# lucagem29/mcmc_clv_model

Hardware: AMD Instinct MI355X
Metric: MCMC sweeps/sec x N_customers (customer-sweeps/s) (higher is better)
Workload: dtype f64

## Files before the change

include/clvmcmc.h:

```cpp
#ifndef CLVMCMC_H
#define CLVMCMC_H

#include <stdint.h>

#ifdef __cplusplus
extern "C" {
#endif

#define CLV_ABI_VERSION 2

#define CLV_BLOCK 256
#define CLV_MAX_K 9
#define CLV_MAX_D 3

enum { CLV_OK = 0, CLV_EINVAL = -1, CLV_EHIP = -2, CLV_ESTATE = -3, CLV_ENOMEM = -4 };
enum { CLV_RNG_PHILOX = 0, CLV_RNG_REPLAY = 1 };
enum { CLV_SINK_FULL = 0, CLV_SINK_SUMMARY = 1, CLV_SINK_NONE = 2, CLV_SINK_SUMMARY_PCT = 3 };

#define CLV_SUMMARY_MU_CAP 0.05
enum {
  CLV_SUM_LAMBDA = 0, CLV_SUM_MU, CLV_SUM_Z, CLV_SUM_LOG_LAMBDA, CLV_SUM_LOG_MU,
  CLV_SUM_LAMBDA2, CLV_SUM_MU2, CLV_SUM_ETA, CLV_SUM_LOG_ETA, CLV_SUM_MU_CAPPED, CLV_SUM_TAU,
  CLV_N_SUM_STATS
};
// ... 69 lines not shown
int clv_clock_probe(clv_sampler* s, double us, double* ghz);
int clv_launch_info(const clv_sampler* s, int64_t* out);
int clv_split_relay_steps(const clv_sampler* s, int32_t* out);
#define CLV_IPC_HANDLE_BYTES 64
int clv_p2p_info(const clv_sampler* s, int64_t* out);
int clv_p2p_export(clv_sampler* s, void* handle);
int clv_p2p_connect(clv_sampler* s, const void* handles, const uint64_t* ptrs);
int clv_p2p_disconnect(clv_sampler* s);
int clv_p2p_set_persistent(clv_sampler* s, int32_t on);
int clv_set_wait_timeout(clv_sampler* s, double ms);
int clv_set_stream(clv_sampler* s, uint64_t stream);
int clv_note_sweeps(clv_sampler* s, int64_t n);

int clv_read_draws(clv_sampler* s, double* level1, double* level2, double* loglik);
int clv_stream_draws(clv_sampler* s, double* level1);
int clv_read_summary(clv_sampler* s, double* sums, int64_t* n_stored);

int clv_get_state(clv_sampler* s, double* lambdas, double* mus, double* hyper);
int clv_set_state(clv_sampler* s, const double* lambdas, const double* mus, const double* hyper,
                  int64_t sweeps_done);

int clv_set_timing(clv_sampler* s, int32_t enable);
int clv_kernel_time(clv_sampler* s, double* sweep_kernel_ms_total, int64_t* sweep_launches,
                    double* hyper_kernel_ms_total, int64_t* hyper_launches);

int clv_debug_host_times(const clv_sampler* s, int64_t* out);
int clv_debug_philox(uint32_t k0, uint32_t k1, const uint32_t* ctr, int64_t n, uint32_t* out);
int clv_debug_variates(uint64_t seed, int32_t chain, uint32_t sweep, int64_t n, int32_t n_steps,
                       float* t_l, float* t_m, float* u_acc, double* u_z, double* u_tau,
                       double* e_alive, double* eta_z, float* log2_u_acc);
int clv_debug_log2u_scan(uint64_t w_begin, uint64_t w_end, double* out);
int clv_debug_t3(const uint32_t* words, int64_t n, int32_t packed, float* t_l, float* t_m);
int clv_debug_level2(int32_t D, int32_t K, const clv_prior* prior, const double* xty,
                     const double* yty, const double* iw_normal, const double* iw_chi2,
                     const double* z, double* beta, double* sigma);
int clv_debug_stamps(clv_sampler* s, uint64_t* out);
int clv_debug_wg_stamps(clv_sampler* s, uint64_t* out);
int clv_debug_hyper_variates(uint64_t seed, int32_t chain, uint32_t sweep, double df, int64_t n,
                             double* chi2, double* normals);
int clv_debug_exp(const double* x, int64_t n, double* out);
int clv_debug_log(const double* x, int64_t n, double* out);
int clv_debug_mh_step(int64_t n, const int32_t* x, const uint8_t* z, const double* T_cal, const double* tau,
                      const double* mean, const double* prec3, const double* cur_pt, const float* t3,
                      const double* scale2, const float* log_u, double* out);
int clv_debug_wg_map(int32_t n_chains, int32_t nb, int32_t n_cu, int32_t* out);
int clv_debug_persist_fits(int64_t grid_wgs, int32_t blocks_per_cu, int32_t n_cu);
int clv_debug_persist_choice(int32_t D, int32_t K, int32_t n_chains, int64_t grid_wgs, int32_t blocks_per_cu,
                             int32_t n_cu);
int clv_debug_split_fits(int32_t n_chains, int32_t nb, int32_t blocks_per_cu, int32_t n_cu);
int clv_debug_split_choice(int32_t n_chains, int32_t nb, int32_t blocks_per_cu, int32_t n_cu);
int clv_debug_split_layout(int32_t n_chains, int32_t nb, int32_t* out);
int clv_debug_split_relay_plan(int32_t S, int32_t R, int32_t* out);
int clv_debug_split_draw_plan(int32_t R, int32_t share, int32_t* out);
int clv_debug_split_stamps(clv_sampler* s, uint64_t* out);

enum { CLV_EXCHANGE_AUTO = 0, CLV_EXCHANGE_P2P = 1, CLV_EXCHANGE_COPY = 2 };
typedef struct clv_group clv_group;
int clv_group_create(clv_sampler* const* shards, int32_t n, int32_t exchange, clv_group** out);
int clv_group_run(clv_group* g, int64_t n_sweeps);
int32_t clv_group_exchange(const clv_group* g);
void clv_group_destroy(clv_group* g);

enum {
  CLV_L1_MEAN_LAMBDA = 0, CLV_L1_LAMBDA_P025, CLV_L1_LAMBDA_P975, CLV_L1_MEAN_MU, CLV_L1_MEAN_MU_CAPPED,
  CLV_L1_MU_P025, CLV_L1_MU_P975, CLV_L1_MEAN_Z, CLV_L1_MEAN_TAU, CLV_L1_MEAN_ETA, CLV_N_L1_STATS
};
int clv_predict(int32_t device, const double* level1, int64_t n_draws, int64_t n, int32_t width,
                const double* T_cal, double T_star, uint64_t seed, int32_t simulate_spend, double sigma_s,
                int64_t* x_future, double* spend_future);
int clv_predict_sampler(clv_sampler* s, double T_star, uint64_t seed, int32_t simulate_spend,
                        double sigma_s, int64_t* x_future, double* spend_future);
int clv_track(int32_t device, const double* level1, int64_t n_draws, int64_t n, int32_t width,
              const double* birth_week, const double* times, int32_t n_times, uint64_t seed,
              double* inc_weekly);
int clv_track_sampler(clv_sampler* s, const double* birth_week, const double* times, int32_t n_times,
                      uint64_t seed, double* inc_weekly);
int clv_level1_summary(int32_t device, const double* level1, int64_t n_draws, int64_t n, int32_t width,
                       double mu_cap, double* out);
int clv_level1_summary_sampler(clv_sampler* s, double mu_cap, double* out);
int clv_chain_total_loglik(int32_t device, const double* level1, int64_t n_draws, int64_t n, int32_t width,
                           const int32_t* x, const double* T_cal, double* mean_total);
int clv_chain_total_loglik_sampler(clv_sampler* s, double* mean_total);

enum {
  CLV_LTV_VALUE_MEAN = 0, CLV_LTV_VALUE_SD, CLV_LTV_VALUE_P025, CLV_LTV_VALUE_P50, CLV_LTV_VALUE_P975,
  CLV_LTV_RESIDUAL_MEAN, CLV_LTV_RESIDUAL_SD, CLV_LTV_RESIDUAL_P025, CLV_LTV_RESIDUAL_P50, CLV_LTV_RESIDUAL_P975,
  CLV_LTV_P_ALIVE, CLV_LTV_LIFETIME_YRS, CLV_LTV_SURVIVAL_1YR, CLV_N_LTV_STATS
};
enum {
  CLV_LTV_DRAW_EQUITY = 0, CLV_LTV_DRAW_VALUE_TOTAL, CLV_LTV_DRAW_N_ALIVE, CLV_LTV_DRAW_MU_SHARE,
  CLV_N_LTV_DRAW_STATS
};
int clv_lifetime_value(int32_t device, const double* level1, int64_t n_draws, int64_t n, int32_t width,
                       const double* monetary , double delta, double horizon ,
                       double value_scale, double periods_per_year, double* out_customers, double* out_draws);
int clv_lifetime_value_sampler(clv_sampler* s, const double* monetary, double delta, double horizon,
                               double value_scale, double periods_per_year, double* out_customers,
                               double* out_draws);
int clv_ltv_info(int64_t* out);

enum {
  CLV_IC_LPPD = 0, CLV_IC_P_WAIC, CLV_IC_ELPD_WAIC, CLV_IC_ELPD_LOO, CLV_IC_P_LOO, CLV_IC_PARETO_K,
  CLV_IC_TAIL_LEN, CLV_N_IC_STATS
};
int clv_pointwise_loglik(int32_t device, const double* level1, int64_t n_draws, int64_t n, int32_t width,
                         const int32_t* x, const double* t_x, const double* T_cal,
// ... 130 lines not shown
```

mcmc_clv_model_amd/_lib.py:

```python
from __future__ import annotations

import ctypes
import os
from ctypes import c_uint8, POINTER, c_char_p, c_double, c_float, c_int32, c_int64, c_uint32, c_uint64, c_void_p

try:
    import torch
except Exception:
    torch = None

LIB_NAME = "libclvmcmc.so"
LIB_PATH = os.environ.get("CLV_LIB_PATH") or os.path.join(os.path.dirname(os.path.abspath(__file__)), LIB_NAME)

ABI_VERSION = 2
BLOCK = 256
MAX_K = 9
MAX_D = 3
RNG_PHILOX, RNG_REPLAY = 0, 1
SINK_FULL, SINK_SUMMARY, SINK_NONE, SINK_SUMMARY_PCT = 0, 1, 2, 3
EXCHANGE_AUTO, EXCHANGE_P2P, EXCHANGE_COPY = 0, 1, 2
SUM_STATS = ("lambda", "mu", "z", "log_lambda", "log_mu", "lambda2", "mu2", "eta", "log_eta", "mu_capped", "tau")
SUMMARY_MU_CAP = 0.05
N_SUM_STATS = len(SUM_STATS)
TAPE_HYPER = 40
# ... 43 lines not shown
    L = ctypes.CDLL(LIB_PATH, mode=ctypes.RTLD_GLOBAL)
    sp = c_void_p
    dp = POINTER(c_double)
    sigs = {
        "clv_abi_version": (c_int32, []),
        "clv_default_blocks_per_unit": (c_int32, [c_int64]),
        "clv_sizeof": (c_int64, [c_int32]),
        "clv_last_error": (c_char_p, []),
        "clv_device_count": (c_int32, [POINTER(c_int32)]),
        "clv_create": (c_int32, [POINTER(ClvConfig), POINTER(ClvData), POINTER(ClvPrior), POINTER(sp)]),
        "clv_destroy": (None, [sp]),
        "clv_set_replay_tape": (c_int32, [sp, dp, c_int64]),
        "clv_replay_sweep_stride": (c_int64, [sp]),
        "clv_run": (c_int32, [sp, c_int64]),
        "clv_rollback": (c_int32, [sp]),
        "clv_sweep": (c_int32, [sp]),
        "clv_hyper": (c_int32, [sp, c_void_p]),
        "clv_partials": (c_int32, [sp, POINTER(c_void_p), POINTER(c_int64), POINTER(c_int32)]),
        "clv_copy_partials": (c_int32, [sp, c_void_p]),
        "clv_synchronize": (c_int32, [sp]),
        "clv_sweeps_done": (c_int64, [sp]),
        "clv_clock_ghz": (c_int32, [sp, POINTER(c_double)]),
        "clv_clock_probe": (c_int32, [sp, c_double, POINTER(c_double)]),
        "clv_launch_info": (c_int32, [sp, POINTER(c_int64)]),
        "clv_split_relay_steps": (c_int32, [sp, POINTER(c_int32)]),
        "clv_p2p_info": (c_int32, [sp, POINTER(c_int64)]),
        "clv_p2p_export": (c_int32, [sp, c_void_p]),
        "clv_p2p_connect": (c_int32, [sp, c_void_p, POINTER(c_uint64)]),
        "clv_p2p_disconnect": (c_int32, [sp]),
        "clv_p2p_set_persistent": (c_int32, [sp, c_int32]),
        "clv_set_wait_timeout": (c_int32, [sp, c_double]),
        "clv_set_stream": (c_int32, [sp, c_uint64]),
        "clv_note_sweeps": (c_int32, [sp, c_int64]),
        "clv_read_draws": (c_int32, [sp, dp, dp, dp]),
        "clv_stream_draws": (c_int32, [sp, dp]),
        "clv_read_summary": (c_int32, [sp, dp, POINTER(c_int64)]),
        "clv_get_state": (c_int32, [sp, dp, dp, dp]),
        "clv_set_state": (c_int32, [sp, dp, dp, dp, c_int64]),
        "clv_set_timing": (c_int32, [sp, c_int32]),
        "clv_kernel_time": (c_int32, [sp, dp, POINTER(c_int64), dp, POINTER(c_int64)]),
        "clv_debug_philox": (c_int32, [c_uint32, c_uint32, POINTER(c_uint32), c_int64, POINTER(c_uint32)]),
        "clv_debug_variates": (c_int32, [c_uint64, c_int32, c_uint32, c_int64, c_int32, POINTER(c_float),
                                         POINTER(c_float), POINTER(c_float), dp, dp, dp, dp, POINTER(c_float)]),
        "clv_debug_log2u_scan": (c_int32, [c_uint64, c_uint64, dp]),
        "clv_debug_host_times": (c_int32, [sp, POINTER(c_int64)]),
        "clv_debug_t3": (c_int32, [POINTER(c_uint32), c_int64, c_int32, POINTER(c_float), POINTER(c_float)]),
        "clv_debug_level2": (c_int32, [c_int32, c_int32, POINTER(ClvPrior), dp, dp, dp, dp, dp, dp, dp]),
        "clv_debug_hyper_variates": (c_int32, [c_uint64, c_int32, c_uint32, c_double, c_int64, dp, dp]),
        "clv_debug_stamps": (c_int32, [sp, POINTER(c_uint64)]),
        "clv_debug_wg_stamps": (c_int32, [sp, POINTER(c_uint64)]),
        "clv_debug_split_stamps": (c_int32, [sp, POINTER(c_uint64)]),
        "clv_debug_split_relay_plan": (c_int32, [c_int32, c_int32, POINTER(c_int32)]),
        "clv_debug_split_draw_plan": (c_int32, [c_int32, c_int32, POINTER(c_int32)]),
        "clv_debug_exp": (c_int32, [dp, c_int64, dp]),
        "clv_debug_log": (c_int32, [dp, c_int64, dp]),
        "clv_debug_mh_step": (c_int32, [c_int64, POINTER(c_int32), POINTER(c_uint8), dp, dp, dp, dp, dp,
                                        POINTER(c_float), dp, POINTER(c_float), dp]),
        "clv_debug_wg_map": (c_int32, [c_int32, c_int32, c_int32, POINTER(c_int32)]),
        "clv_debug_persist_choice": (c_int32, [c_int32, c_int32, c_int32, c_int64, c_int32, c_int32]),
        "clv_debug_persist_fits": (c_int32, [c_int64, c_int32, c_int32]),
        "clv_group_create": (c_int32, [POINTER(sp), c_int32, c_int32, POINTER(sp)]),
        "clv_group_run": (c_int32, [sp, c_int64]),
        "clv_group_exchange": (c_int32, [sp]),
        "clv_group_destroy": (None, [sp]),
        "clv_predict": (c_int32, [c_int32, dp, c_int64, c_int64, c_int32, dp, c_double, c_uint64, c_int32, c_double,
                                  POINTER(c_int64), dp]),
        "clv_predict_sampler": (c_int32, [sp, c_double, c_uint64, c_int32, c_double, POINTER(c_int64), dp]),
        "clv_track": (c_int32, [c_int32, dp, c_int64, c_int64, c_int32, dp, dp, c_int32, c_uint64, dp]),
        "clv_track_sampler": (c_int32, [sp, dp, dp, c_int32, c_uint64, dp]),
        "clv_level1_summary": (c_int32, [c_int32, dp, c_int64, c_int64, c_int32, c_double, dp]),
        "clv_level1_summary_sampler": (c_int32, [sp, c_double, dp]),
        "clv_chain_total_loglik": (c_int32, [c_int32, dp, c_int64, c_int64, c_int32, POINTER(c_int32), dp, dp]),
        "clv_chain_total_loglik_sampler": (c_int32, [sp, dp]),
        "clv_lifetime_value": (c_int32, [c_int32, dp, c_int64, c_int64, c_int32, dp, c_double, c_double, c_double,
                                         c_double, dp, dp]),
        "clv_lifetime_value_sampler": (c_int32, [sp, dp, c_double, c_double, c_double, c_double, dp, dp]),
        "clv_ltv_info": (c_int32, [POINTER(c_int64)]),
        "clv_pointwise_loglik": (c_int32, [c_int32, dp, c_int64, c_int64, c_int32, POINTER(c_int32), dp, dp, dp,
                                           c_double, dp]),
        "clv_psis_loo": (c_int32, [c_int32, dp, c_int64, c_int64, c_double, dp]),
        "clv_information_criteria": (c_int32, [c_int32, dp, c_int64, c_int64, c_int32, POINTER(c_int32), dp, dp, dp,
                                               c_double, c_double, dp]),
        "clv_information_criteria_sampler": (c_int32, [sp, c_int32, c_double, c_double, dp]),
        "clv_ic_info": (c_int32, [POINTER(c_int64)]),
        "clv_debug_information_criteria": (c_int32, [c_int32, dp, c_int64, c_int64, c_int32, POINTER(c_int32), dp,
                                                     dp, dp, c_double, c_double, c_int64, c_int32, dp]),
        "clv_score_customers": (c_int32, [c_int32, c_int32, c_int32, c_int32, c_int64, dp, c_int64, POINTER(c_int32), dp,
                                          dp, dp, dp, c_double, c_int32, c_int32, c_int32, c_uint64, c_int32, c_int64,
                                          c_int64, dp, dp, c_int32, dp, dp, dp, dp]),
        "clv_score_customers_sampler": (c_int32, [sp, c_int64, POINTER(c_int32), dp, dp, dp, dp, c_int32, c_int32,
                                                  c_int32, c_uint64, c_int64, c_int64, dp, dp, c_int32, dp, dp, dp, dp]),
        "clv_score_info": (c_int32, [POINTER(c_int64)]),
        "clv_debug_score_hyper": (c_int32, [c_int32, c_int32, c_int32, c_int64, dp, c_double, dp]),
        "clv_forecast": (c_int32, [c_int32, dp, c_int64, c_int64, c_int32, POINTER(c_int32), dp, dp, c_double, c_int32,
                                   POINTER(c_int32), dp, dp]),
        "clv_forecast_sampler": (c_int32, [sp, c_double, c_int32, POINTER(c_int32), dp, dp]),
        "clv_forecast_info": (c_int32, [POINTER(c_int64)]),
        "clv_debug_forecast": (c_int32, [c_int32, dp, c_int64, c_int64, c_int32, POINTER(c_int32), dp, dp, c_double,
                                         c_int32, POINTER(c_int32), c_int64, c_int32, dp, dp]),
        "clv_ppc": (c_int32, [c_int32, c_int32, dp, c_int32, dp, c_int32, c_int32, dp, c_int64, c_int64,
                              POINTER(c_int32), dp, dp, c_int32, c_uint64, c_int64, dp, POINTER(c_int64), dp,
                              POINTER(c_int64), dp]),
        "clv_ppc_sampler": (c_int32, [sp, c_int32, c_int32, c_uint64, dp, POINTER(c_int64), dp, POINTER(c_int64), dp]),
        "clv_ppc_info": (c_int32, [POINTER(c_int64)]),
        "clv_debug_ppc": (c_int32, [c_int32, c_int32, dp, c_int32, dp, c_int32, c_int32, dp, c_int64, c_int64,
                                    POINTER(c_int32), dp, dp, c_int32, c_uint64, c_int64, dp, POINTER(c_int64), dp,
# ... 151 lines not shown
```

mcmc_clv_model_amd/csrc/capi.hip:

```cpp
#include <hip/hip_runtime.h>

#include <algorithm>
#include <chrono>
#include <cstdlib>
#include <cstdio>
#include <cstring>
#include <string>
#include <vector>

#include "internal.h"
#include "kernels.h"
#include "philox.h"

using namespace clv;

namespace {

thread_local std::string g_err;

constexpr int PRIOR_DOUBLES = 81 + 81 + 27 + 9;
constexpr int GRAPH_CHUNK = 64;
constexpr int TIMING_EVENTS = 256;

}
// ... 1553 lines not shown
  CLV_HIP(dalloc(&dc, n));
  CLV_HIP(dalloc(&dn, n));
  CLV_HIP(launch_debug_hyper_variates(seed, chain, sweep, df, n, dc, dn, nullptr));
  CLV_HIP(hipMemcpy(chi2, dc, sizeof(double) * n, hipMemcpyDeviceToHost));
  CLV_HIP(hipMemcpy(normals, dn, sizeof(double) * n, hipMemcpyDeviceToHost));
  CLV_HIP(hipFree(dc));
  CLV_HIP(hipFree(dn));
  return CLV_OK;
}

int clv_debug_persist_choice(int32_t D, int32_t K, int32_t n_chains, int64_t grid_wgs, int32_t blocks_per_cu,
                             int32_t n_cu) {
  return persist_grid_fits(grid_wgs, blocks_per_cu, n_cu) && persist_worth(D, K, n_chains, grid_wgs, n_cu) ? 1 : 0;
}

int clv_debug_persist_fits(int64_t grid_wgs, int32_t blocks_per_cu, int32_t n_cu) {
  return persist_grid_fits(grid_wgs, blocks_per_cu, n_cu) ? 1 : 0;
}

int clv_debug_split_fits(int32_t n_chains, int32_t nb, int32_t blocks_per_cu, int32_t n_cu) {
  return persist_split_fits(n_chains, nb, blocks_per_cu, n_cu) ? 1 : 0;
}

int clv_debug_split_choice(int32_t n_chains, int32_t nb, int32_t blocks_per_cu, int32_t n_cu) {
  return persist_split_fits(n_chains, nb, blocks_per_cu, n_cu) && persist_split_pays(n_chains, nb, n_cu) ? 1 : 0;
}

int clv_debug_split_relay_plan(int32_t S, int32_t R, int32_t* out) {
  if (!out || S < 0 || S > PRE_STEPS || !(R == 0 || R == 8 || R == 12)) return fail(CLV_EINVAL, "bad arguments");
  const SplitRelayPlan pl = split_relay_plan(S, R);
  const int32_t o[8] = {pl.own_begin, pl.own_end, pl.relay_begin, pl.relay_end,
                        pl.own_begin, pl.own_end, pl.relay_begin, pl.relay_end};
  std::copy(o, o + 8, out);
  return CLV_OK;
}

int clv_debug_split_draw_plan(int32_t R, int32_t share, int32_t* out) {
  if (!out || !(R == 8 || R == 12) || share < -1 || share >= SPLIT_DRAW_SHARES) return fail(CLV_EINVAL, "bad arguments");
  if (share < 0) {
    out[0] = SPLIT_RELAY_DRAW;
    return CLV_OK;
  }
  constexpr int NQ = PRE_STEPS / 4;
  for (int row = 0; row < SPLIT_CW; ++row) {
    for (int q = 0; q < NQ; ++q) {
      const SplitDrawSlot d = split_draw_plan(R, share, row, q);
      const int32_t o[4] = {d.wave, d.slot, d.staged, d.reader};
      std::copy(o, o + 4, out + (row * NQ + q) * 4);
    }
  }
  return CLV_OK;
}

int clv_debug_split_layout(int32_t n_chains, int32_t nb, int32_t* out) {
  if (!out || n_chains < 1 || nb < 1 || nb > SPLIT_MAX_NB || n_chains >= (1 << 15)) return fail(CLV_EINVAL, "bad arguments");
  const std::vector<int32_t> m = persist_split_layout(n_chains, nb);
  const int nwg = split_wgs(nb);
  for (size_t i = 0; i < m.size(); ++i) {
    int32_t* o = out + 8 * i;
    const int p = m[i] & 0xFFFF;
    o[0] = m[i] >> 16;
    for (int k = 1; k < 8; ++k) o[k] = -1;
    if (p == nwg) continue;
    const int r0 = SPLIT_CW * p;
    o[1] = r0;
    o[2] = std::min(SPLIT_CW, 4 * nb - r0);
    const int b0 = (p & 1) ? (r0 - 2) / 4 : r0 / 4, b1 = (p & 1) ? (r0 + 2) / 4 : r0 / 4 + 1;
    o[3] = (p & 1) ? 3 : 1;
    o[4] = b0;
    if (b1 < nb) {
      o[5] = (p & 1) ? 1 : 2;
      o[6] = b1;
    }
    o[7] = (p & 1) ? nb + 2 * (b0 / 3) : -1;
  }
  return CLV_OK;
}

int clv_debug_wg_map(int32_t n_chains, int32_t nb, int32_t n_cu, int32_t* out) {
  if (!out || n_chains < 1 || nb < 0 || n_cu < 1 || n_chains >= (1 << 15) || nb >= (1 << 16))
    return fail(CLV_EINVAL, "bad arguments");
  const std::vector<int32_t> m = persist_wg_map(n_chains, nb, n_cu);
  std::copy(m.begin(), m.end(), out);
  return CLV_OK;
}

int clv_debug_mh_step(int64_t n, const int32_t* x, const uint8_t* z, const double* T_cal, const double* tau,
                      const double* mean, const double* prec3, const double* cur_pt, const float* t3,
                      const double* scale2, const float* log_u, double* out) {
  if (!x || !z || !T_cal || !tau || !mean || !prec3 || !cur_pt || !t3 || !scale2 || !log_u || !out || n < 1)
    return fail(CLV_EINVAL, "bad arguments");
  int32_t *dx;
  uint8_t* dz;
  double *dT, *dtau, *dm, *dp, *dc, *ds, *dout;
  float *dt3, *dlu;
  CLV_HIP(hipMalloc(&dx, sizeof(int32_t) * n));
  CLV_HIP(hipMalloc(&dz, n));
  CLV_HIP(dalloc(&dT, n));
  CLV_HIP(dalloc(&dtau, n));
  CLV_HIP(dalloc(&dm, 2 * n));
  CLV_HIP(dalloc(&dp, 3));
  CLV_HIP(dalloc(&dc, 2 * n));
  CLV_HIP(dalloc(&ds, 2));
  CLV_HIP(dalloc(&dout, 7 * n));
  CLV_HIP(hipMalloc(&dt3, sizeof(float) * 2 * n));
  CLV_HIP(hipMalloc(&dlu, sizeof(float) * n));
// ... 38 lines not shown
```

mcmc_clv_model_amd/csrc/kernels.h:

```cpp
#pragma once
#include <hip/hip_runtime.h>
#include <stdint.h>

#include "../../include/clvmcmc.h"

namespace clv {

constexpr int BLOCK = CLV_BLOCK;
constexpr int HS = 64;
constexpr int H_TAG = 63;
constexpr int TAPE_HYPER = 40;
constexpr int MAX_WORLD = 64;
constexpr int UMAIL = 2048;
constexpr int HV = 40;
constexpr int MAIL_TAIL = MAX_WORLD;
constexpr int CLK_RING = 1024;
constexpr int DIAG_WORDS = 16;
constexpr int PRE_STEPS = 20;
constexpr int SPLIT_CW = 6;
constexpr int SPLIT_NT = 512;
constexpr int SPLIT_MAX_NB = 256;
enum : int { LAYOUT_NONE = 0, LAYOUT_BLOCK = 1, LAYOUT_SPLIT = 2 };
__host__ __device__ inline int split_wgs(int nb) { return (2 * nb + 2) / 3; }
__host__ __device__ inline int split_records(int nb) { return nb + 2 * ((nb + 1) / 3); }
enum : int { WAIT_HYPER = 1, WAIT_BLOCKS = 2, WAIT_P2P_MAIL = 3, WAIT_FX_MAIL = 4, WAIT_RELAY = 5 };
#ifndef CLV_SPLIT_RELAY_STEPS
#define CLV_SPLIT_RELAY_STEPS 8
#endif
constexpr int SPLIT_RELAY_STEPS = CLV_SPLIT_RELAY_STEPS;
static_assert(SPLIT_RELAY_STEPS == 0 || SPLIT_RELAY_STEPS == 8 || SPLIT_RELAY_STEPS == 12, "relay point: 8 or 12 steps");
struct SplitRelayPlan {
  int own_begin, own_end, relay_begin, relay_end;
};
__host__ __device__ constexpr SplitRelayPlan split_relay_plan(int S, int R) {
  return SplitRelayPlan{0, (R > 0 && S > R) ? R : S, (R > 0 && S > R) ? R : S, S};
}
#ifndef CLV_SPLIT_RELAY_DRAW
#define CLV_SPLIT_RELAY_DRAW 4
#endif
#ifndef CLV_SPLIT_RELAY_GAP2_CHUNKS
#define CLV_SPLIT_RELAY_GAP2_CHUNKS 3
#endif
#ifndef CLV_SPLIT_RELAY_GAP2_STOP
#define CLV_SPLIT_RELAY_GAP2_STOP 6
#endif
constexpr int SPLIT_RELAY_DRAW = CLV_SPLIT_RELAY_DRAW;
constexpr int SPLIT_RELAY_GAP2_CHUNKS = CLV_SPLIT_RELAY_GAP2_CHUNKS;
constexpr int SPLIT_RELAY_GAP2_STOP = CLV_SPLIT_RELAY_GAP2_STOP;
constexpr int SPLIT_DRAW_SHARES = 6;
static_assert(SPLIT_RELAY_DRAW >= 0 && SPLIT_RELAY_DRAW < SPLIT_DRAW_SHARES, "draw share: 0..5");
static_assert(SPLIT_RELAY_GAP2_CHUNKS >= 1 && SPLIT_RELAY_GAP2_STOP >= 1 && SPLIT_RELAY_GAP2_STOP <= SPLIT_CW, "gap 2 limits");
enum : int { DRAW_WINDOW = 0, DRAW_GAP1 = 1, DRAW_GAP2 = 2 };
struct SplitDrawSlot {
  int wave;
  int slot;
  int staged;
  int reader;
};
__host__ __device__ constexpr int split_draw_gap1_chunks(int share) { return share >= 4 ? share - 3 : share >= 2 ? share - 1 : 0; }
__host__ __device__ constexpr SplitDrawSlot split_draw_plan(int R, int share, int row, int chunk) {
  const int qr = R / 4;
  const int reader = (row >= 4 && chunk >= qr) ? row + 2 : row;
  if (share >= 1 && share <= 3 && row >= 4 && chunk >= qr && chunk < qr + SPLIT_RELAY_GAP2_CHUNKS)
    return SplitDrawSlot{row + 2, DRAW_GAP2, 0, reader};
  if ((row & 3) < 2 && chunk < split_draw_gap1_chunks(share) && chunk < qr)
    return SplitDrawSlot{6 + (row & 1), DRAW_GAP1, 1, reader};
  return SplitDrawSlot{reader, DRAW_WINDOW, 0, reader};
}

__host__ __device__ inline int64_t mail_slots(int world, int chains, int stride, int units_per_rank) {
  return 2LL * world * chains * stride * units_per_rank;
}

enum : int {
  H_BETA = 0,
  H_SIGMA = 27,
  H_P00 = 36, H_P01 = 37, H_P11 = 38,
  H_S00 = 39, H_S11 = 40,
  H_S22 = 41, H_POSTVAR = 42, H_SQRT_POSTVAR = 43, H_OMEGA2 = 44,
  H_INV_OMEGA2 = 45, H_INV_S22 = 46,
};

struct Ctrl {
  int64_t cur;
  uint32_t arrive;
  uint32_t abort;
};

struct Geometry {
  int D, K, S;
  int n_chains;
  int64_t n;
  int64_t n_global;
  int64_t shard_begin;
  int nb_local;
  int blocks_per_rank;
  int blocks_per_unit;
  int units_per_rank;
  int64_t n_units_global;
  int world_size;
  int stride;
  int burnin, mcmc, thin, n_draws;
  int l2w;
};

struct Rng {
  uint64_t seed;
  int chain_first;
  const double* tape;
  int64_t tape_sweep_stride;
  int64_t tape_sweeps;
};

struct HyperArgs {
  Geometry g;
  Rng r;
  const double* units;
  double* hyper;
  Ctrl* ctrl;
  double* level2;
// ... 107 lines not shown
```

mcmc_clv_model_amd/csrc/kernels.hip:

```cpp
#include <hip/hip_ext.h>

#include "fastmath.h"
#include "internal.h"
#include "kernels.h"
#include "philox.h"

#ifndef SWEEP_MH_PIPELINE
#define SWEEP_MH_PIPELINE 1
#endif
#ifndef CLV_OPAQUE_GI
#define CLV_OPAQUE_GI(D) ((D) == 3)
#endif
#ifndef CLV_L2_OPAQUE
#define CLV_L2_OPAQUE(P) (P)
#endif
#ifndef CLV_L2_LANE0_MAX
#define CLV_L2_LANE0_MAX 6
#endif
#ifndef PERSIST_REDUCE_GEN
#define PERSIST_REDUCE_GEN 1
#endif
#ifndef SWEEP_REDUCE_CHUNK
#define SWEEP_REDUCE_CHUNK 8
#endif
// ... 1335 lines not shown
      float u[MC];
#pragma unroll
      for (int st = 0; st < MC; ++st) {
        t[st] = v.t[(q * MC + st) * NT + v.lane];
        u[st] = v.u[(q * MC + st) * NT + v.lane];
      }
#pragma unroll
      for (int st = 0; st < MC; ++st) mh_step(cu, s00, s11, t[st].x, t[st].y, u[st], exp_tab);
    }
  }
}

template <int Q0, int Q1, int NT>
__device__ __forceinline__ void mh_pre_variates_range(const SlotPhilox& ph, int S_, const PreVariates& v) {
  constexpr int MC = MH_CHUNK_STEPS;
  const int S = opaque_uniform(S_);
#pragma unroll
  for (int q = Q0; q < Q1; ++q) {
    if (q * MC < S) {
      float tl[MC], tm[MC], lu[MC];
      mh_chunk_variates(ph, (uint32_t)q, tl, tm, lu);
#pragma unroll
      for (int st = 0; st < MC; ++st) {
        const int k = q * MC + st;
        v.t[k * NT + v.lane] = make_float2(tl[st], tm[st]);
        v.u[k * NT + v.lane] = k < S ? lu[st] : __builtin_inff();
      }
    }
  }
}
template <int Q0, int Q1, int NT, int NS, bool COPY>
__device__ __forceinline__ void mh_pre_variates_window(const SlotPhilox& ph, int S_, const PreVariates& v,
                                                       const PreVariates& sv, uint32_t have) {
  constexpr int MC = MH_CHUNK_STEPS;
  const int S = opaque_uniform(S_);
  have = (uint32_t)__builtin_amdgcn_readfirstlane((int)have);
#pragma unroll
  for (int q = Q0; q < Q1; ++q) {
    if (q * MC < S) {
      if ((have >> q) & 1u) {
        if constexpr (COPY) {
          float2 t[MC];
          float u[MC];
#pragma unroll
          for (int st = 0; st < MC; ++st) {
            t[st] = sv.t[(q * MC + st) * NS + sv.lane];
            u[st] = sv.u[(q * MC + st) * NS + sv.lane];
          }
#pragma unroll
          for (int st = 0; st < MC; ++st) {
            v.t[(q * MC + st) * NT + v.lane] = t[st];
            v.u[(q * MC + st) * NT + v.lane] = u[st];
          }
        }
      } else {
        float tl[MC], tm[MC], lu[MC];
        mh_chunk_variates(ph, (uint32_t)q, tl, tm, lu);
#pragma unroll
        for (int st = 0; st < MC; ++st) {
          const int k = q * MC + st;
          v.t[k * NT + v.lane] = make_float2(tl[st], tm[st]);
          v.u[k * NT + v.lane] = k < S ? lu[st] : __builtin_inff();
        }
      }
    }
  }
}
template <int Q0, int Q1, int NT, int D, int K, bool CL>
__device__ __forceinline__ void mh_run_pre_range(Cust<D, K, CL>& cu, const PreVariates& v, double s00, double s11, int S,
                                                 const double* exp_tab) {
  constexpr int MC = MH_CHUNK_STEPS;
  S = opaque_uniform(S);
#pragma unroll
  for (int q = Q0; q < Q1; ++q) {
    if (q * MC < S) {
      float2 t[MC];
      float u[MC];
#pragma unroll
      for (int st = 0; st < MC; ++st) {
        t[st] = v.t[(q * MC + st) * NT + v.lane];
        u[st] = v.u[(q * MC + st) * NT + v.lane];
      }
#pragma unroll
      for (int st = 0; st < MC; ++st) mh_step(cu, s00, s11, t[st].x, t[st].y, u[st], exp_tab);
    }
  }
}

template <int D>
struct CustOut {
  double lam, mu, eta, lgl, lgm, leta;
};

__device__ __forceinline__ double eta_normal(uint32_t k0, uint32_t k1, uint32_t gi, int64_t s, const double* tab) {
  const u32x4 r = customer_block(k0, k1, gi, (uint32_t)s, SLOT_ETA);
  return sqrt(-2.0 * log_fast(u53_open0(r.x, r.y), tab)) * cos2pi_u53(r.z, r.w, tab);
}

template <int D, int K, bool REPLAY, bool CL>
__device__ __forceinline__ CustOut<D> cust_finish(Cust<D, K, CL>& u, const SweepArgs& a, int64_t s, bool stored,
                                                  const double* H, uint32_t k0, uint32_t k1, const double* tape,
                                                  const double* exp_tab, StatGen<D, K>& st,
                                                  const double* zeta_pre = nullptr) {
  const Geometry& g = a.g;
  const int64_t i = u.i;
  double lam, mu;
// ... 926 lines not shown
    }
    CLV_P_STAMP(a.stamps, wgi, 6, stp);
  }
  if (cu.active) {
    const int64_t ci = (int64_t)c * g.n + cu.i;
    a.lam_out[ci] = cu.lam;
    a.mu_out[ci] = cu.mu;
  }
}

#ifndef CLV_SPLIT_HELP_CHUNKS
#define CLV_SPLIT_HELP_CHUNKS 2
#endif
constexpr int SPLIT_NC = SPLIT_CW * 64;
constexpr int SPLIT_PRE_LDS_BYTES = PRE_STEPS * SPLIT_NC * 12;

constexpr int RELAY_REC = 11;

template <int D, int K, int R>
__device__ __forceinline__ void split_relay_sweeps(const SweepArgs& a_launch, int64_t s_first, int64_t n_sweeps, int c,
                                                   int p, uint32_t k0, uint32_t k1, int64_t wgi, int64_t it_stamp,
                                                   double* parts, char* pool, double (*red)[K * D + D * (D + 1) / 2 + 1],
                                                   const double* exp_tab, double* Hs, uint32_t* s_abort) {
  constexpr int NS = K * D + D * (D + 1) / 2 + 1;
  constexpr int MC = MH_CHUNK_STEPS;
  constexpr int NQ = PRE_STEPS / MC;
  static_assert(R > 0 && R % MC == 0 && R < PRE_STEPS, "relay point: whole chunks, inside the pool");
  constexpr SplitRelayPlan PLAN = split_relay_plan(PRE_STEPS, R);
  static_assert(PLAN.own_begin == 0 && PLAN.own_end == PLAN.relay_begin && PLAN.own_end % MC == 0 && PLAN.relay_end == PRE_STEPS,
                "the relay plan cuts between chunks");
  static_assert(split_relay_plan(R + 1, R).own_end == PLAN.own_end, "one cut for every relayed S");
  constexpr int QR = PLAN.relay_begin / MC;
  __shared__ double relay_rec[RELAY_REC][128];
  __shared__ double relay_ret[4][128];
  __shared__ uint32_t relay_flag[2];
  __shared__ uint32_t relay_abort;
  (void)wgi;
  (void)it_stamp;
  const int tid = threadIdx.x;
  const int wave = __builtin_amdgcn_readfirstlane(tid >> 6);
  const bool first_wait = a_launch.pend_in != nullptr;
  if (tid < 2) relay_flag[tid] = 0;
  if (tid == 2) relay_abort = 0;
  constexpr int DRAW = SPLIT_RELAY_DRAW;
  constexpr int HC1 = split_draw_gap1_chunks(DRAW);
  constexpr bool GAP2 = split_draw_plan(R, DRAW, 4, QR).slot == DRAW_GAP2;
  static_assert(HC1 <= QR, "gap 1 draws owner chunks only");
  static_assert(HC1 == 0 || (split_draw_plan(R, DRAW, 0, HC1 - 1).wave == SPLIT_CW && split_draw_plan(R, DRAW, 4, HC1 - 1).wave == SPLIT_CW &&
                             split_draw_plan(R, DRAW, 1, HC1 - 1).wave == SPLIT_CW + 1 && split_draw_plan(R, DRAW, 5, HC1 - 1).wave == SPLIT_CW + 1 &&
                             split_draw_plan(R, DRAW, 0, HC1).slot == DRAW_WINDOW && split_draw_plan(R, DRAW, 2, 0).slot == DRAW_WINDOW),
                "gap 1: the first HC1 chunks of rows 0 and 4 by wavefront 6, of rows 1 and 5 by wavefront 7");
  static_assert(GAP2 == (split_draw_plan(R, DRAW, 5, QR).slot == DRAW_GAP2) && split_draw_plan(R, DRAW, 4, QR - 1).slot != DRAW_GAP2,
                "gap 2: the relay wavefront's own chunks, the same of rows 4 and 5");
  constexpr int STAGE_STEPS = (HC1 > 0 ? HC1 : 1) * MC;
  float2* stage_t = nullptr;
  float* stage_u = nullptr;
  uint32_t* relay_drawn = nullptr;
  uint32_t* relay_arrive = nullptr;
  if constexpr (HC1 > 0) {
    __shared__ __attribute__((aligned(16))) char stage[4 * STAGE_STEPS * 64 * 12];
    __shared__ uint32_t drawn[4];
    stage_t = (float2*)stage;
    stage_u = (float*)(stage + 4 * STAGE_STEPS * 64 * 8);
    relay_drawn = drawn;
  }
  if constexpr (GAP2) {
    __shared__ uint32_t arrive;
    relay_arrive = &arrive;
    if (tid == 3) arrive = 0;
  }

  if (wave >= SPLIT_CW) {
    const int rw = wave - SPLIT_CW;
    const int rl = tid - SPLIT_CW * 64;
    const PreVariates pv{(float2*)pool, (float*)(pool + PRE_STEPS * SPLIT_NC * 8), tid - 128};
    Cust<D, K> cu;
    {
      const Geometry& g = a_launch.g;
      const int64_t i = (int64_t)p * SPLIT_NC + (tid - 128);
      cu.active = i < g.n;
      cu.i = cu.active ? i : (g.n > 0 ? g.n - 1 : 0);
      cu.xr_[0] = 1.0;
#pragma unroll
      for (int k = 1; k < K; ++k) cu.xr_[k] = a_launch.cov[(int64_t)(k - 1) * g.n + cu.i];
      cu.gi = (uint32_t)(g.shard_begin + cu.i);
      cu.xm = 0.0;
      cu.lc.omz = 0.0;
      if (cu.active) mh_pre_variates_range<QR, NQ, SPLIT_NC>(SlotPhilox(k0, k1, cu.gi, (uint32_t)s_first), g.S, pv);
    }
    __syncthreads();
    for (int64_t it = 0; it < n_sweeps; ++it) {
      const SweepArgs& a = loop_args<CLV_PERSIST_FRESH_ARGS != 0>(a_launch);
      const Geometry& g = a.g;
      if (it > 0 || first_wait) {
        __syncthreads();
        if (*s_abort) return;
      }
      const int64_t s = uniform64(s_first + it);
      const bool stored = is_stored(s, g);
      const uint32_t tag = (uint32_t)it + 1u;
      const bool ahead = it + 1 < n_sweeps;
      if constexpr (HC1 > 0) {
        if (ahead) {
          const int S = opaque_uniform(g.S);
          uint32_t have[2] = {0u, 0u};
          bool go = true;
#pragma unroll
          for (int q = 0; q < HC1; ++q) {
#pragma unroll
            for (int t = 0; t < 2; ++t) {
              if (q * MC < S) {
                if (go)
                  go = (uint32_t)__builtin_amdgcn_readfirstlane(
                           (int)__hip_atomic_load(&relay_flag[rw], __ATOMIC_RELAXED, __HIP_MEMORY_SCOPE_WORKGROUP)) != tag;
                if (go) {
                  const int64_t i = (int64_t)p * SPLIT_NC + (rw + 4 * t) * 64 + (tid & 63);
                  if (i < g.n) {
                    const SlotPhilox ph(k0, k1, (uint32_t)(g.shard_begin + i), (uint32_t)(s + 1));
                    float tl[MC], tm[MC], lu[MC];
                    mh_chunk_variates(ph, (uint32_t)q, tl, tm, lu);
                    const int col = ((2 * t + rw) * STAGE_STEPS + q * MC) * 64 + (tid & 63);
#pragma unroll
                    for (int st = 0; st < MC; ++st) {
                      stage_t[col + st * 64] = make_float2(tl[st], tm[st]);
                      stage_u[col + st * 64] = q * MC + st < S ? lu[st] : __builtin_inff();
                    }
                  }
                  have[t] |= 1u << q;
                }
              }
            }
          }
          if ((tid & 63) == 0) {
            relay_drawn[rw] = have[0];
            relay_drawn[2 + rw] = have[1];
          }
        }
        CLV_R_STAMP(a, wgi, 12 + rw, it == it_stamp);
      }
      bool seen = true;
      {
        const uint64_t t0 = __builtin_amdgcn_s_memrealtime();
        for (uint32_t poll = 0;; ++poll) {
          const uint32_t f = (uint32_t)__builtin_amdgcn_readfirstlane(
              (int)__hip_atomic_load(&relay_flag[rw], __ATOMIC_RELAXED, __HIP_MEMORY_SCOPE_WORKGROUP));
          if (f == tag) break;
          const int ws = wait_state(a, t0, poll, a.wait_ticks);
          if (ws != WAIT_GOING) {
            if (ws == WAIT_EXPIRED) {
              report_wait(a, WAIT_RELAY, s, c, false, p, 4 + rw, f, poll, t0);
              raise_abort(a);
            }
            if ((tid & 63) == 0) relay_abort = 1;
            seen = false;
            break;
          }
          __builtin_amdgcn_s_sleep(1);
        }
      }
      __builtin_amdgcn_fence(__ATOMIC_ACQUIRE, "workgroup", "local");
      CLV_R_STAMP(a, wgi, 2 * rw, it == it_stamp);
      StatGen<D, K> st{};
      __builtin_amdgcn_s_setprio(3);
// ... 96 lines not shown
    const bool stp = tid == 0 && it == it_stamp;
    (void)stp;
    CLV_P_STAMP(a.stamps, wgi, 0, stp);
    if (it > 0 || first_wait) {
      if (tid < 64) {
        const double* src = hyp_c + (int64_t)(s & 1) * g.n_chains * HS;
        const uint64_t t0 = __builtin_amdgcn_s_memrealtime();
        for (uint32_t poll = 0;; ++poll) {
          const double v = ld_wt(src + tid);
          if (__all(slot_full(v))) {
            Hs[tid] = v;
            break;
          }
          const int ws = wait_state(a, t0, poll, hyper_wait_ticks(a));
          if (ws != WAIT_GOING) {
            if (ws == WAIT_EXPIRED) {
              report_wait(a, WAIT_HYPER, s, c, slot_full(v), p, tid, dbits(v), poll, t0);
              raise_abort(a);
            }
            if (tid == 0) *s_abort = 1;
            break;
          }
          __builtin_amdgcn_s_sleep(1);
        }
      }
      __syncthreads();
      if (*s_abort) return;
    }
    CLV_P_STAMP(a.stamps, wgi, 1, stp);
    StatGen<D, K> st{};
    CustOut<D> out{};
    if (relayed) {
      __builtin_amdgcn_s_setprio(3);
      if (cu.active) {
        cust_coeffs<D, K, false>(cu, Hs, exp_tab);
        mh_run_pre_range<0, QR, SPLIT_NC>(cu, pv, Hs[H_S00], Hs[H_S11], g.S, exp_tab);
        relay_rec[0][rl] = cu.fc.A;
        relay_rec[1][rl] = cu.fc.B;
        relay_rec[2][rl] = cu.fc.C;
        relay_rec[3][rl] = cu.fc.Dl;
        relay_rec[4][rl] = cu.fc.El;
        relay_rec[5][rl] = cu.fc.w;
        relay_rec[6][rl] = cu.ll;
        relay_rec[7][rl] = cu.lm;
        relay_rec[8][rl] = cu.cur;
        if (stored) {
          relay_rec[9][rl] = cu.xm;
          relay_rec[10][rl] = cu.lc.omz;
        }
      }
      __builtin_amdgcn_fence(__ATOMIC_RELEASE, "workgroup", "local");
      if ((tid & 63) == 0)
        __hip_atomic_store(&relay_flag[wave - 4], (uint32_t)it + 1u, __ATOMIC_RELAXED, __HIP_MEMORY_SCOPE_WORKGROUP);
    } else {
      __builtin_amdgcn_s_setprio(2);
      if (cu.active) {
        cust_coeffs<D, K, false>(cu, Hs, exp_tab);
        CLV_P_STAMP(a.stamps, wgi, 2, stp);
        mh_run_pre_range<0, QR, SPLIT_NC>(cu, pv, Hs[H_S00], Hs[H_S11], g.S, exp_tab);
        mh_run_pre_range<QR, NQ, SPLIT_NC>(cu, pv, Hs[H_S00], Hs[H_S11], g.S, exp_tab);
        CLV_P_STAMP(a.stamps, wgi, 3, stp);
        out = cust_finish<D, K, false>(cu, a, s, stored, Hs, k0, k1, nullptr, exp_tab, st, nullptr);
      }
      CLV_P_STAMP(a.stamps, wgi, 4, stp);
      wave_reduce_gen<NS, SWEEP_REDUCE_CHUNK>(st, red);
    }
    if constexpr (GAP2) {
      if ((tid & 63) == 0) __hip_atomic_fetch_add(relay_arrive, 1u, __ATOMIC_RELAXED, __HIP_MEMORY_SCOPE_WORKGROUP);
    }
    __syncthreads();
    if (relay_abort) return;
    {
      const int j = tid & 63;
      const int r0 = SPLIT_CW * p;
      if (j < NS && tid < 128) {
        if ((p & 1) == 0) {
          if (tid < 64) {
            st_wt(parts + (int64_t)(r0 / 4) * NS + j, ((red[0][j] + red[1][j]) + red[2][j]) + red[3][j]);
          } else {
            const int b = r0 / 4 + 1;
            if (b < g.nb_local) st_wt(parts + (int64_t)b * NS + j, red[4][j] + red[5][j]);
          }
        } else {
          if (tid < 64) {
            const int b = (r0 - 2) / 4;
            double* ext = parts + (int64_t)(g.nb_local + 2 * (b / 3)) * NS;
            st_wt(ext + j, red[0][j]);
            st_wt(ext + NS + j, red[1][j]);
          } else {
            const int b = (r0 + 2) / 4;
            if (b < g.nb_local) st_wt(parts + (int64_t)b * NS + j, ((red[2][j] + red[3][j]) + red[4][j]) + red[5][j]);
          }
        }
      }
    }
    __builtin_amdgcn_s_setprio(0);
    CLV_P_STAMP(a.stamps, wgi, 5, stp);
    CLV_P_STAMP(a.stamps, wgi, 8, stp);
    CLV_P_STAMP(a.stamps, wgi, 9, stp);
#ifdef CLV_STAMPS
    if (stp && a.stamps) a.stamps[1024 * 8 + wgi * 12 + 11] = blockIdx.y * gridDim.x + blockIdx.x;
#endif
    if (cu.active) {
      if (relayed) {
        cu.lam = relay_ret[0][rl];
        cu.mu = relay_ret[1][rl];
        out = CustOut<D>{cu.lam, cu.mu, 1.0, relay_ret[2][rl], relay_ret[3][rl], 0.0};
      }
      cust_store<D, K>(cu, out, a, c, s, stored, false);
      if (it + 1 < n_sweeps) {
        cust_ztau<D, K, false>(cu, a, s + 1, k0, k1, nullptr, exp_tab);
        const SlotPhilox ph(k0, k1, cu.gi, (uint32_t)(s + 1));
        if constexpr (HC1 > 0) {
          const int w = __builtin_amdgcn_readfirstlane(tid >> 6);
          const int sr = 2 * (w >> 2) + (w & 1);
          const uint32_t have = (w & 3) < 2 ? relay_drawn[sr] : 0u;
          const PreVariates sv{stage_t + sr * STAGE_STEPS * 64, stage_u + sr * STAGE_STEPS * 64, tid & 63};
          mh_pre_variates_window<0, HC1, SPLIT_NC, 64, true>(ph, g.S, pv, sv, have);
          mh_pre_variates_range<HC1, QR, SPLIT_NC>(ph, g.S, pv);
        } else {
          mh_pre_variates_range<0, QR, SPLIT_NC>(ph, g.S, pv);
        }
        if (!relayed) mh_pre_variates_range<QR, NQ, SPLIT_NC>(ph, g.S, pv);
      }
    }
    CLV_P_STAMP(a.stamps, wgi, 6, stp);
  }
  if (cu.active) {
    const int64_t ci = (int64_t)c * a_launch.g.n + cu.i;
    a_launch.lam_out[ci] = cu.lam;
    a_launch.mu_out[ci] = cu.mu;
  }
}

template <int D, int K, int HC, int R = 0>
__global__ __launch_bounds__(SPLIT_NT, 1) void persist_kernel_split(SweepArgs a, int64_t s_first, int64_t n_sweeps) {
  static_assert(D == 2, "the split layout is bivariate");
  constexpr int NXY = K * D;
  constexpr int NYY = D * (D + 1) / 2;
  constexpr int NS = NXY + NYY + 1;
  constexpr int MC = MH_CHUNK_STEPS;
  constexpr int NQ = PRE_STEPS / MC;
  static_assert(HC >= 0 && HC <= NQ, "helper share");
  __shared__ double red[SPLIT_CW][NS];
  __shared__ __attribute__((aligned(16))) double exp_tab[FAST_TAB_N];
  __shared__ double Hs[HS];
  __shared__ uint32_t s_abort;
  __shared__ __attribute__((aligned(16))) char pool[SPLIT_PRE_LDS_BYTES];
  const Geometry& g = a.g;
  const int nwg = split_wgs(g.nb_local);
  int c = blockIdx.y, p = blockIdx.x;
  if (a.wg_map) {
    const int32_t m = a.wg_map[blockIdx.y * gridDim.x + blockIdx.x];
    c = m >> 16;
    p = m & 0xFFFF;
  }
  const int tid = threadIdx.x;
  const int wave = __builtin_amdgcn_readfirstlane(tid >> 6);
  const int64_t wgi = (int64_t)c * (nwg + 1) + p;
  const int64_t it_stamp = n_sweeps >= 2 ? n_sweeps - 2 : 0;
  (void)wgi;
  (void)it_stamp;
  uint32_t k0, k1;
  chain_key(a.r.seed, (int64_t)a.r.chain_first + c, &k0, &k1);
  double* parts = a.pblock + (int64_t)c * split_records(g.nb_local) * NS;
  if (tid == 0) s_abort = 0;
// ... 741 lines not shown
```

Baseline: 11.50 billion.

## Let relay owner waves pre-draw their last variate chunks after publishing

Adds an owner-gap draw plan: once the relay wavefronts have published their relay results, they generate the last few next-sweep MH variate chunks for their own rows, which the main path then skips through an in-pool mask. An optional mode limits gap-1 staging to rows 0/1, which shrinks the shared-memory staging buffer. The aim is to use idle relay-wave time so the critical-path post-store variate generation gets shorter. It adds constexpr plan logic, static asserts and a debug export, and costs extra per-wave work and scheduling complexity.

Result: no change. 11.55 billion (median of 6 runs) (+0.4%).

```diff
diff --git a/include/clvmcmc.h b/include/clvmcmc.h
--- a/include/clvmcmc.h
+++ b/include/clvmcmc.h
@@ -145,6 +145,7 @@
 int clv_debug_split_layout(int32_t n_chains, int32_t nb, int32_t* out);
 int clv_debug_split_relay_plan(int32_t S, int32_t R, int32_t* out);
 int clv_debug_split_draw_plan(int32_t R, int32_t share, int32_t* out);
+int clv_debug_split_draw_plan_ext(int32_t R, int32_t share, int32_t owner, int32_t gap1_rows, int32_t* out);
 int clv_debug_split_stamps(clv_sampler* s, uint64_t* out);
 
 enum { CLV_EXCHANGE_AUTO = 0, CLV_EXCHANGE_P2P = 1, CLV_EXCHANGE_COPY = 2 };
diff --git a/mcmc_clv_model_amd/_lib.py b/mcmc_clv_model_amd/_lib.py
--- a/mcmc_clv_model_amd/_lib.py
+++ b/mcmc_clv_model_amd/_lib.py
@@ -119,6 +119,7 @@
         "clv_debug_split_stamps": (c_int32, [sp, POINTER(c_uint64)]),
         "clv_debug_split_relay_plan": (c_int32, [c_int32, c_int32, POINTER(c_int32)]),
         "clv_debug_split_draw_plan": (c_int32, [c_int32, c_int32, POINTER(c_int32)]),
+        "clv_debug_split_draw_plan_ext": (c_int32, [c_int32, c_int32, c_int32, c_int32, POINTER(c_int32)]),
         "clv_debug_exp": (c_int32, [dp, c_int64, dp]),
         "clv_debug_log": (c_int32, [dp, c_int64, dp]),
         "clv_debug_mh_step": (c_int32, [c_int64, POINTER(c_int32), POINTER(c_uint8), dp, dp, dp, dp, dp,
diff --git a/mcmc_clv_model_amd/csrc/capi.hip b/mcmc_clv_model_amd/csrc/capi.hip
--- a/mcmc_clv_model_amd/csrc/capi.hip
+++ b/mcmc_clv_model_amd/csrc/capi.hip
@@ -1629,6 +1629,26 @@
   return CLV_OK;
 }
 
+int clv_debug_split_draw_plan_ext(int32_t R, int32_t share, int32_t owner, int32_t gap1_rows, int32_t* out) {
+  if (!out || !(R == 8 || R == 12) || share < -1 || share >= SPLIT_DRAW_SHARES) return fail(CLV_EINVAL, "bad arguments");
+  if (share < 0) {
+    out[0] = SPLIT_RELAY_DRAW;
+    out[1] = SPLIT_OWNER_DRAW;
+    out[2] = SPLIT_GAP1_ROWS;
+    return CLV_OK;
+  }
+  if (owner < 0 || owner > SPLIT_OWNER_DRAW_MAX || gap1_rows < 0 || gap1_rows > 1) return fail(CLV_EINVAL, "bad arguments");
+  constexpr int NQ = PRE_STEPS / 4;
+  for (int row = 0; row < SPLIT_CW; ++row) {
+    for (int q = 0; q < NQ; ++q) {
+      const SplitDrawSlot d = split_draw_plan_ext(R, share, owner, gap1_rows, row, q);
+      const int32_t o[4] = {d.wave, d.slot, d.staged, d.reader};
+      std::copy(o, o + 4, out + (row * NQ + q) * 4);
+    }
+  }
+  return CLV_OK;
+}
+
 int clv_debug_split_layout(int32_t n_chains, int32_t nb, int32_t* out) {
   if (!out || n_chains < 1 || nb < 1 || nb > SPLIT_MAX_NB || n_chains >= (1 << 15)) return fail(CLV_EINVAL, "bad arguments");
   const std::vector<int32_t> m = persist_split_layout(n_chains, nb);
diff --git a/mcmc_clv_model_amd/csrc/kernels.h b/mcmc_clv_model_amd/csrc/kernels.h
--- a/mcmc_clv_model_amd/csrc/kernels.h
+++ b/mcmc_clv_model_amd/csrc/kernels.h
@@ -66,6 +66,31 @@
   if ((row & 3) < 2 && chunk < split_draw_gap1_chunks(share) && chunk < qr)
     return SplitDrawSlot{6 + (row & 1), DRAW_GAP1, 1, reader};
   return SplitDrawSlot{reader, DRAW_WINDOW, 0, reader};
+}
+#ifndef CLV_SPLIT_OWNER_DRAW
+#define CLV_SPLIT_OWNER_DRAW 1
+#endif
+#ifndef CLV_SPLIT_GAP1_ROWS
+#define CLV_SPLIT_GAP1_ROWS 0
+#endif
+constexpr int SPLIT_OWNER_DRAW = CLV_SPLIT_OWNER_DRAW;
+constexpr int SPLIT_GAP1_ROWS = CLV_SPLIT_GAP1_ROWS;
+constexpr int SPLIT_OWNER_DRAW_MAX = 2;
+static_assert(SPLIT_OWNER_DRAW >= 0 && SPLIT_OWNER_DRAW <= SPLIT_OWNER_DRAW_MAX, "owner gap: 0, 1 or 2 chunks");
+static_assert(SPLIT_GAP1_ROWS == 0 || SPLIT_GAP1_ROWS == 1, "gap 1 rows: 0 (r and r + 4) or 1 (0 / 1 only)");
+enum : int { DRAW_OWNER = 3 };
+__host__ __device__ constexpr SplitDrawSlot split_draw_plan_ext(int R, int share, int owner, int gap1_rows, int row, int chunk) {
+  const int qr = R / 4;
+  const SplitDrawSlot d = split_draw_plan(R, share, row, chunk);
+  const bool gap1 = d.slot == DRAW_GAP1 && !(gap1_rows == 1 && row >= 4);
+  if (row >= 4 && chunk < qr && chunk >= qr - owner && !gap1) return SplitDrawSlot{row, DRAW_OWNER, 0, row};
+  if (d.slot == DRAW_GAP1 && !gap1) return SplitDrawSlot{d.reader, DRAW_WINDOW, 0, d.reader};
+  return d;
+}
+__host__ __device__ constexpr int split_owner_first_chunk(int R, int share, int owner, int gap1_rows) {
+  int q = R / 4;
+  while (q > 0 && split_draw_plan_ext(R, share, owner, gap1_rows, 4, q - 1).slot == DRAW_OWNER) --q;
+  return q;
 }
 
 __host__ __device__ inline int64_t mail_slots(int world, int chains, int stride, int units_per_rank) {
diff --git a/mcmc_clv_model_amd/csrc/kernels.hip b/mcmc_clv_model_amd/csrc/kernels.hip
--- a/mcmc_clv_model_amd/csrc/kernels.hip
+++ b/mcmc_clv_model_amd/csrc/kernels.hip
@@ -1411,6 +1411,42 @@
             v.t[(q * MC + st) * NT + v.lane] = t[st];
             v.u[(q * MC + st) * NT + v.lane] = u[st];
           }
+        }
+      } else {
+        float tl[MC], tm[MC], lu[MC];
+        mh_chunk_variates(ph, (uint32_t)q, tl, tm, lu);
+#pragma unroll
+        for (int st = 0; st < MC; ++st) {
+          const int k = q * MC + st;
+          v.t[k * NT + v.lane] = make_float2(tl[st], tm[st]);
+          v.u[k * NT + v.lane] = k < S ? lu[st] : __builtin_inff();
+        }
+      }
+    }
+  }
+}
+template <int Q0, int Q1, int HC, int NT, int NS>
+__device__ __forceinline__ void mh_pre_variates_window_ext(const SlotPhilox& ph, int S_, const PreVariates& v,
+                                                           const PreVariates& sv, uint32_t have, uint32_t inpool) {
+  constexpr int MC = MH_CHUNK_STEPS;
+  const int S = opaque_uniform(S_);
+  have = (uint32_t)__builtin_amdgcn_readfirstlane((int)have);
+  inpool = (uint32_t)__builtin_amdgcn_readfirstlane((int)inpool);
+#pragma unroll
+  for (int q = Q0; q < Q1; ++q) {
+    if (q * MC < S && !((inpool >> q) & 1u)) {
+      if (q < HC && ((have >> q) & 1u)) {
+        float2 t[MC];
+        float u[MC];
+#pragma unroll
+        for (int st = 0; st < MC; ++st) {
+          t[st] = sv.t[(q * MC + st) * NS + sv.lane];
+          u[st] = sv.u[(q * MC + st) * NS + sv.lane];
+        }
+#pragma unroll
+        for (int st = 0; st < MC; ++st) {
+          v.t[(q * MC + st) * NT + v.lane] = t[st];
+          v.u[(q * MC + st) * NT + v.lane] = u[st];
         }
       } else {
         float tl[MC], tm[MC], lu[MC];
@@ -2443,16 +2479,34 @@
                 "gap 1: the first HC1 chunks of rows 0 and 4 by wavefront 6, of rows 1 and 5 by wavefront 7");
   static_assert(GAP2 == (split_draw_plan(R, DRAW, 5, QR).slot == DRAW_GAP2) && split_draw_plan(R, DRAW, 4, QR - 1).slot != DRAW_GAP2,
                 "gap 2: the relay wavefront's own chunks, the same of rows 4 and 5");
+  constexpr int OWN = SPLIT_OWNER_DRAW;
+  constexpr int G1R = SPLIT_GAP1_ROWS;
+  constexpr bool EXT = OWN > 0 || G1R > 0;
+  constexpr int G1T = G1R ? 1 : 2;
+  constexpr int HC1O = G1R ? 0 : HC1;
+  constexpr int OQ0 = split_owner_first_chunk(R, DRAW, OWN, G1R);
+  static_assert(OQ0 >= HC1O && OQ0 <= QR && (OWN > 0 || OQ0 == QR) && QR - OQ0 <= OWN,
+                "owner gap: the owner's last chunks, above those gap 1 may take for its row");
+  static_assert((OQ0 == QR || (split_draw_plan_ext(R, DRAW, OWN, G1R, 4, OQ0).wave == 4 && split_draw_plan_ext(R, DRAW, OWN, G1R, 5, OQ0).wave == 5 &&
+                               split_draw_plan_ext(R, DRAW, OWN, G1R, 5, QR - 1).slot == DRAW_OWNER &&
+                               split_draw_plan_ext(R, DRAW, OWN, G1R, 0, OQ0).slot != DRAW_OWNER)) &&
+                    (OQ0 == 0 || split_draw_plan_ext(R, DRAW, OWN, G1R, 5, OQ0 - 1).slot != DRAW_OWNER) &&
+                    split_draw_plan_ext(R, DRAW, OWN, G1R, 4, QR).slot != DRAW_OWNER,
+                "owner gap: rows 4 and 5 by their owners, the same chunks of both");
+  static_assert(HC1 == 0 || ((split_draw_plan_ext(R, DRAW, OWN, G1R, 4, 0).slot == DRAW_GAP1) == (G1R == 0) &&
+                             split_draw_plan_ext(R, DRAW, OWN, G1R, 0, 0).slot == DRAW_GAP1 && split_draw_plan_ext(R, DRAW, OWN, G1R, 1, 0).slot == DRAW_GAP1),
+                "gap 1: rows 4 / 5 only with CLV_SPLIT_GAP1_ROWS = 0");
   constexpr int STAGE_STEPS = (HC1 > 0 ? HC1 : 1) * MC;
+  constexpr int STAGE_ROWS = 2 * G1T;
   float2* stage_t = nullptr;
   float* stage_u = nullptr;
   uint32_t* relay_drawn = nullptr;
   uint32_t* relay_arrive = nullptr;
   if constexpr (HC1 > 0) {
-    __shared__ __attribute__((aligned(16))) char stage[4 * STAGE_STEPS * 64 * 12];
+    __shared__ __attribute__((aligned(16))) char stage[STAGE_ROWS * STAGE_STEPS * 64 * 12];
     __shared__ uint32_t drawn[4];
     stage_t = (float2*)stage;
-    stage_u = (float*)(stage + 4 * STAGE_STEPS * 64 * 8);
+    stage_u = (float*)(stage + STAGE_ROWS * STAGE_STEPS * 64 * 8);
     relay_drawn = drawn;
   }
   if constexpr (GAP2) {
@@ -2499,7 +2553,7 @@
 #pragma unroll
           for (int q = 0; q < HC1; ++q) {
 #pragma unroll
-            for (int t = 0; t < 2; ++t) {
+            for (int t = 0; t < G1T; ++t) {
               if (q * MC < S) {
                 if (go)
                   go = (uint32_t)__builtin_amdgcn_readfirstlane(
@@ -2702,6 +2756,12 @@
       __builtin_amdgcn_fence(__ATOMIC_RELEASE, "workgroup", "local");
       if ((tid & 63) == 0)
         __hip_atomic_store(&relay_flag[wave - 4], (uint32_t)it + 1u, __ATOMIC_RELAXED, __HIP_MEMORY_SCOPE_WORKGROUP);
+      if constexpr (OQ0 < QR) {
+        __builtin_amdgcn_s_setprio(0);
+        if (cu.active && it + 1 < n_sweeps)
+          mh_pre_variates_range<OQ0, QR, SPLIT_NC>(SlotPhilox(k0, k1, cu.gi, (uint32_t)(s + 1)), g.S, pv);
+        if constexpr (!GAP2) CLV_R_STAMP(a, wgi, 14 + (wave - 4), it == it_stamp);
+      }
     } else {
       __builtin_amdgcn_s_setprio(2);
       if (cu.active) {
@@ -2761,7 +2821,18 @@
       if (it + 1 < n_sweeps) {
         cust_ztau<D, K, false>(cu, a, s + 1, k0, k1, nullptr, exp_tab);
         const SlotPhilox ph(k0, k1, cu.gi, (uint32_t)(s + 1));
-        if constexpr (HC1 > 0) {
+        if constexpr (EXT) {
+          const int w = __builtin_amdgcn_readfirstlane(tid >> 6);
+          uint32_t have = 0u, inpool = 0u;
+          PreVariates sv = pv;
+          if constexpr (HC1 > 0) {
+            const int sr = (G1R ? 0 : 2 * (w >> 2)) + (w & 1);
+            if ((w & 3) < 2 && (G1R == 0 || w < 4)) have = relay_drawn[sr];
+            sv = PreVariates{stage_t + sr * STAGE_STEPS * 64, stage_u + sr * STAGE_STEPS * 64, tid & 63};
+          }
+          if (relayed) inpool = ((1u << QR) - 1u) & ~((1u << OQ0) - 1u);
+          mh_pre_variates_window_ext<0, QR, HC1, SPLIT_NC, 64>(ph, g.S, pv, sv, have, inpool);
+        } else if constexpr (HC1 > 0) {
           const int w = __builtin_amdgcn_readfirstlane(tid >> 6);
           const int sr = 2 * (w >> 2) + (w & 1);
           const uint32_t have = (w & 3) < 2 ? relay_drawn[sr] : 0u;
```
